# ur-whitelab/nmrgnn

Hardware: AMD Instinct MI355X
Metric: atoms/s (fwd+bwd) on 256-atom/16-neighbor synthetic graphs (higher is better)
Workload: dtype f32 (2xf16-piece MFMA, f32 accumulate)

## Files before the change

include/nmrgnn_hip.h:

```cpp
#ifndef NMRGNN_HIP_H
#define NMRGNN_HIP_H

#include <stdint.h>

#ifdef __cplusplus
extern "C" {
#endif

#define NG_ABI_VERSION 9

enum {
  NG_OK = 0,
  NG_ERR_INVALID = -1,
  NG_ERR_HIP = -2,
  NG_ERR_NOMEM = -3,
  NG_ERR_UNSUPPORTED = -4
};

enum { NG_ACT_NONE = 0, NG_ACT_SOFTPLUS = 1, NG_ACT_RELU = 2, NG_ACT_TANH = 3 };

typedef struct ng_ctx ng_ctx;

int ng_abi_version(void);
int ng_ctx_create(int device, ng_ctx** out);
// ... 78 lines not shown
                const float* dd, float scale, int G, const int32_t* graph_ptr, const float* box, int triclinic, double* strain,
                double* dvec);
int ng_box_grad_csr(ng_ctx*, void* stream, int64_t N, int64_t nnz, const float* pos, const int32_t* row_ptr,
                    const int32_t* col, const float* dd, float scale, int G, const int32_t* graph_ptr, const float* box,
                    int triclinic, double* strain, double* dvec);

int ng_embed_fwd(ng_ctx*, void* stream, int64_t N, int C, int F, const float* atoms,
                 const float* Wemb, float* h0);
int ng_embed_bwd(ng_ctx*, void* stream, int64_t N, int C, int F, const float* atoms,
                 const float* dh0, float* dWemb);

int ng_mp_aggregate(ng_ctx*, void* stream, int64_t N, int K, int F, int E, const float* h,
                    const int32_t* nlist, const float* e, float* A);

int ng_mp_layer_fwd(ng_ctx*, void* stream, int64_t N, int K, int F, int E, int act, int residual,
                    const float* h, const int32_t* nlist, const float* e, const float* inv_degree,
                    const float* w, float* h_out, float* A_save, float* s_save);
int ng_mp_layer_wants_aggregate(int F, int E, int K);

int ng_mp_layer_bwd(ng_ctx*, void* stream, int64_t N, int K, int F, int E, int act,
                    const float* h, const int32_t* nlist, const float* e, const float* inv_degree,
                    const float* w, const float* A_save, const float* s_save,
                    const int32_t* csc_ptr, const int32_t* csc_edge, const float* dh_out,
                    float* dh_in, float* de, int de_accum, float* dw);

int ng_mp_edge_records(ng_ctx*, void* stream, int64_t N, int K, int E, const int32_t* csc_ptr,
                       const int32_t* csc_edge, const float* e, float* rec);
int ng_mp_layer_bwd_rec(ng_ctx*, void* stream, int64_t N, int K, int F, int E, int act,
                    const float* h, const int32_t* nlist, const float* e, const float* inv_degree,
                    const float* w, const float* A_save, const float* s_save,
                    const int32_t* csc_ptr, const int32_t* csc_edge, const float* dh_out,
                    float* dh_in, float* de, int de_accum, float* dw, const float* csc_rec);

int ng_mp_aggregate_csr(ng_ctx*, void* stream, int64_t N, int F, int E, const float* h,
                        const int32_t* row_ptr, const int32_t* col, const float* e, float* A);
int ng_mp_layer_fwd_csr(ng_ctx*, void* stream, int64_t N, int64_t nnz, int F, int E, int act, int residual,
                        const float* h, const int32_t* row_ptr, const int32_t* col, const float* e,
                        const float* inv_degree, const float* w, float* h_out, float* A_save, float* s_save);
int ng_mp_layer_bwd_csr(ng_ctx*, void* stream, int64_t N, int64_t nnz, int F, int E, int act, const float* h,
                        const int32_t* row_ptr, const int32_t* col, const int32_t* row_of, const float* e,
                        const float* inv_degree, const float* w, const float* A_save, const float* s_save,
                        const int32_t* csc_ptr, const int32_t* csc_edge, const float* dh_out, float* dh_in,
                        float* de, int de_accum, float* dw);

int ng_mp_layer_fwd_short(ng_ctx*, void* stream, int64_t N, int K, int F, int E, int act, int residual, const float* h,
                          const int32_t* nlist, const float* e, const float* inv_degree, const float* w, float* h_out);
int ng_mp_layer_fwd_short_csr(ng_ctx*, void* stream, int64_t N, int F, int E, int act, int residual, const float* h,
                              const int32_t* row_ptr, const int32_t* col, const float* e, const float* inv_degree,
                              const float* w, float* h_out);
int ng_mp_layer_short_ok(int64_t N, int K, int F, int E);
int ng_fc_head_ok(int64_t N, int F, int L, int C, int act);
int ng_fc_head_fwd(ng_ctx*, void* stream, int64_t N, int F, int L, int C, int act, const float* x,
                   const float* const* W, const float* const* b, const float* Wout, const float* bout,
                   const float* atoms, const float* pstd, const float* pavg, float* peaks);

int ng_build_incoming_lists(ng_ctx*, void* stream, int64_t N, int K, int64_t n_entries, const int32_t* nlist,
                            const float* edges, int32_t* nlist_c, int32_t* csc_ptr, int32_t* csc_edge);
size_t ng_incoming_lists_scratch_bytes(int64_t N, int64_t n_entries);

int ng_cutoff_count(ng_ctx*, void* stream, int G, int n, float cutoff, const float* pos, int32_t* deg);
int ng_cutoff_fill(ng_ctx*, void* stream, int G, int n, float cutoff, float scale, const float* pos,
                   const int32_t* row_ptr, int32_t* col, float* dist, float* inv_degree);
int ng_cutoff_fill_rows(ng_ctx*, void* stream, int G, int n, float cutoff, float scale, const float* pos,
                        const int32_t* row_ptr, int32_t* col, float* dist, float* inv_degree, int32_t* row_of);
int ng_cutoff_count_pbc(ng_ctx*, void* stream, int G, int n, float cutoff, const float* pos, const float* box, int triclinic,
                        int32_t* deg);
// ... 100 lines not shown
```

nmrgnn_amd/_lib.py:

```python
from __future__ import annotations

import ctypes as C
import os
import threading

_HERE = os.path.dirname(os.path.abspath(__file__))
LIB_PATH = os.environ.get("NMRGNN_HIP_LIB") or os.path.join(_HERE, "csrc", "libnmrgnn_hip.so")

NG_ACT_NONE, NG_ACT_SOFTPLUS, NG_ACT_RELU, NG_ACT_TANH = 0, 1, 2, 3
ACT_CODES = {None: NG_ACT_NONE, "linear": NG_ACT_NONE, "softplus": NG_ACT_SOFTPLUS, "relu": NG_ACT_RELU,
             "tanh": NG_ACT_TANH}

_c_float_p = C.POINTER(C.c_float)
_c_int32_p = C.POINTER(C.c_int32)
_vp = C.c_void_p
_i64 = C.c_int64
_u64 = C.c_uint64
_int = C.c_int
_f = C.c_float

SIGNATURES = {
    "ng_abi_version": (_int, []),
    "ng_ctx_create": (_int, [_int, C.POINTER(_vp)]),
    "ng_ctx_destroy": (None, [_vp]),
# ... 27 lines not shown
    "ng_edge_table_scatter": (_int, [_vp, _vp, _i64, _int, _int, _int, _vp, _vp, _vp, _vp, _vp, _vp]),
    "ng_edge_mlp_bwd": (_int, [_vp, _vp, _i64, _int, _int, _int, _int, _vp, _vp, _vp, _f,
                               C.POINTER(_vp), _vp, _vp, C.POINTER(_vp), C.POINTER(_vp)]),
    "ng_edge_mlp_bwd_tape": (_int, [_vp, _vp, _i64, _int, _int, _int, _int, _vp, _vp, _vp, _f,
                                    C.POINTER(_vp), _vp, _vp, C.POINTER(_vp), C.POINTER(_vp), _int]),
    "ng_build_live_edges": (_int, [_vp, _vp, _i64, _vp, _vp, _vp, _vp, _vp]),
    "ng_build_graph_lists": (_int, [_vp, _vp, _i64, _int, _vp, _vp, _vp, _vp, _vp, _vp, _vp, _vp, _vp]),
    "ng_graph_lists_one_launch": (_int, [_i64, _int]),
    "ng_add_noise_live": (_int, [_vp, _vp, _u64, _u64, _i64, _vp, _vp, _f, _vp, _vp]),
    "ng_edge_live_supported": (_int, [_int, _int, _int, _int]),
    "ng_edge_mlp_fwd_live": (_int, [_vp, _vp, _i64, _int, _int, _int, _int, _vp, _vp, _vp, _vp, _vp, _f,
                                    C.POINTER(_vp), C.POINTER(_vp), _vp, _vp]),
    "ng_edge_mlp_bwd_live": (_int, [_vp, _vp, _i64, _int, _int, _int, _int, _vp, _vp, _vp, _vp, _vp, _f,
                                    C.POINTER(_vp), _vp, _vp, C.POINTER(_vp), C.POINTER(_vp), _int]),
    "ng_edge_mlp_dinput": (_int, [_vp, _vp, _i64, _int, _int, _int, _int, _vp, _vp, _vp, _vp, _vp, _f,
                                  C.POINTER(_vp), C.POINTER(_vp), _vp, _vp, _vp]),
    "ng_positions_grad": (_int, [_vp, _vp, _i64, _int, _vp, _vp, _vp, _vp, _f, _vp, _vp, _vp]),
    "ng_positions_grad_csr": (_int, [_vp, _vp, _i64, _i64, _vp, _vp, _vp, _vp, _vp, _f, _vp, _vp, _vp]),
    "ng_positions_grad_pbc": (_int, [_vp, _vp, _i64, _int, _vp, _vp, _vp, _vp, _f, _vp, _vp, _int, _vp, _int, _vp]),
    "ng_positions_grad_csr_pbc": (_int, [_vp, _vp, _i64, _i64, _vp, _vp, _vp, _vp, _vp, _f, _vp, _vp, _int, _vp, _int, _vp]),
    "ng_box_grad": (_int, [_vp, _vp, _i64, _int, _vp, _vp, _vp, _vp, _f, _int, _vp, _vp, _int, _vp, _vp]),
    "ng_box_grad_csr": (_int, [_vp, _vp, _i64, _i64, _vp, _vp, _vp, _vp, _f, _int, _vp, _vp, _int, _vp, _vp]),
    "ng_restraint_loss": (_int, [_vp, _vp, _int, _i64, _vp, _vp, _vp, _vp, _vp]),
    "ng_restraint_loss_ex": (_int, [_vp, _vp, _int, _i64, _int, _vp, _vp, _vp, _vp, _vp, _f, _vp, _vp, _vp, _vp]),
    "ng_embed_fwd": (_int, [_vp, _vp, _i64, _int, _int, _vp, _vp, _vp]),
    "ng_embed_bwd": (_int, [_vp, _vp, _i64, _int, _int, _vp, _vp, _vp]),
    "ng_mp_aggregate": (_int, [_vp, _vp, _i64, _int, _int, _int, _vp, _vp, _vp, _vp]),
    "ng_mp_layer_fwd": (_int, [_vp, _vp, _i64, _int, _int, _int, _int, _int, _vp, _vp, _vp, _vp, _vp,
                               _vp, _vp, _vp]),
    "ng_mp_layer_bwd": (_int, [_vp, _vp, _i64, _int, _int, _int, _int, _vp, _vp, _vp, _vp, _vp,
                               _vp, _vp, _vp, _vp, _vp, _vp, _vp, _int, _vp]),
    "ng_mp_layer_bwd_rec": (_int, [_vp, _vp, _i64, _int, _int, _int, _int, _vp, _vp, _vp, _vp, _vp,
                               _vp, _vp, _vp, _vp, _vp, _vp, _vp, _int, _vp, _vp]),
    "ng_mp_edge_records": (_int, [_vp, _vp, _i64, _int, _int, _vp, _vp, _vp, _vp]),
    "ng_mp_aggregate_csr": (_int, [_vp, _vp, _i64, _int, _int, _vp, _vp, _vp, _vp, _vp]),
    "ng_mp_layer_fwd_csr": (_int, [_vp, _vp, _i64, _i64, _int, _int, _int, _int, _vp, _vp, _vp, _vp, _vp, _vp,
                                   _vp, _vp, _vp]),
    "ng_mp_layer_bwd_csr": (_int, [_vp, _vp, _i64, _i64, _int, _int, _int, _vp, _vp, _vp, _vp, _vp, _vp, _vp,
                                   _vp, _vp, _vp, _vp, _vp, _vp, _vp, _int, _vp]),
    "ng_build_incoming_lists": (_int, [_vp, _vp, _i64, _int, _i64, _vp, _vp, _vp, _vp, _vp]),
    "ng_incoming_lists_scratch_bytes": (C.c_size_t, [_i64, _i64]),
    "ng_cutoff_count": (_int, [_vp, _vp, _int, _int, _f, _vp, _vp]),
    "ng_cutoff_fill": (_int, [_vp, _vp, _int, _int, _f, _f, _vp, _vp, _vp, _vp, _vp]),
    "ng_cutoff_fill_rows": (_int, [_vp, _vp, _int, _int, _f, _f, _vp, _vp, _vp, _vp, _vp, _vp]),
    "ng_cutoff_count_pbc": (_int, [_vp, _vp, _int, _int, _f, _vp, _vp, _int, _vp]),
    "ng_cutoff_fill_rows_pbc": (_int, [_vp, _vp, _int, _int, _f, _f, _vp, _vp, _int, _vp, _vp, _vp, _vp, _vp]),
    "ng_exclusive_scan_i32": (_int, [_vp, _vp, _i64, _vp, _vp]),
    "ng_dense_fwd": (_int, [_vp, _vp, _i64, _int, _int, _int, _int, _vp, _vp, _vp, _vp, _vp]),
    "ng_dense_bwd": (_int, [_vp, _vp, _i64, _int, _int, _int, _int, _vp, _vp, _vp, _vp, _vp, _vp,
                            _vp]),
    "ng_head_fwd": (_int, [_vp, _vp, _i64, _int, _int, _vp, _vp, _vp, _vp, _vp, _vp, _vp, _vp]),
    "ng_head_fwd_dropout": (_int, [_vp, _vp, _i64, _int, _int, _vp, _u64, _u64, _f, _vp, _vp, _vp, _vp, _vp, _vp, _vp]),
    "ng_head_bwd": (_int, [_vp, _vp, _i64, _int, _int, _vp, _vp, _vp, _vp, _vp, _vp, _vp, _vp, _vp]),
    "ng_head_loss_blocks": (_int, [_vp, _int, _int, _int, _i64]),
    "ng_head_loss_bwd": (_int, [_vp, _vp, _i64, _int, _int, _int, _i64, _vp, _u64, _u64, _f, _vp, _vp, _vp, _vp, _vp, _vp, _vp,
                               _vp, _vp, _f, _vp, _vp, _vp]),
    "ng_head_loss_reduce": (_int, [_vp, _vp, _vp, _int, _int, _int, _vp, _vp, _vp]),
    "ng_mp_layer_wants_aggregate": (_int, [_int, _int, _int]),
    "ng_fc_block_fwd": (_int, [_vp, _vp, _i64, _int, _int, _int, _vp, _vp, _vp, _vp, _vp]),
    "ng_fc_block_scratch_floats": (_i64, [_i64, _int, _int]),
    "ng_fc_block_bwd": (_int, [_vp, _vp, _i64, _int, _int, _int, _vp, _vp, _vp, _vp, _vp, _vp, _vp, _vp]),
    "ng_mp_layer_fwd_short": (_int, [_vp, _vp, _i64, _int, _int, _int, _int, _int, _vp, _vp, _vp, _vp, _vp, _vp]),
    "ng_mp_layer_fwd_short_csr": (_int, [_vp, _vp, _i64, _int, _int, _int, _int, _vp, _vp, _vp, _vp, _vp, _vp, _vp]),
    "ng_mp_layer_short_ok": (_int, [_i64, _int, _int, _int]),
    "ng_fc_head_ok": (_int, [_i64, _int, _int, _int, _int]),
    "ng_fc_head_fwd": (_int, [_vp, _vp, _i64, _int, _int, _int, _int, _vp, C.POINTER(_vp), C.POINTER(_vp), _vp, _vp, _vp,
# ... 119 lines not shown
```

nmrgnn_amd/engine.py:

```python
from __future__ import annotations

import ctypes as C
import os

import numpy as np
import torch

from . import _lib
from ._lib import ptr, ptr_array
from .graph import GraphBatch
from .params import ParamStore

ACT = {None: 0, "linear": 0, "softplus": 1, "relu": 2, "tanh": 3}
DROPOUT_RATE = 0.2
FUSED_TAIL_MAX_ATOMS = 16384


def rbf_grid(low, high, count):
    lo, hi = np.float32(low), np.float32(high)
    delta = (hi - lo) / np.float32(count - 1)
    c = (lo + delta * np.arange(count, dtype=np.float32)).astype(np.float32)
    c[-1] = hi
    return c, float(np.float32(c[1] - c[0]))


def edge_path(edge_table, use_live_edges, live_kernels, E, n_edges, min_edges, is_csr, capturing):
    fits = n_edges * E * 4 < (1 << 31)
    sized = edge_table and E <= 8 and n_edges >= min_edges and fits
    if live_kernels and fits:
        return "table" if sized else ("live" if use_live_edges else "slots")
    if sized and not is_csr and not capturing:
        return "table_host"
    return "slots"


class Tape:
    __slots__ = ("batch", "d_eff", "z_save", "z_layout", "e", "h", "A", "S", "fx", "g", "drop_mask",
                 "peaks", "edge_path", "live", "table", "loss", "dpeaks", "dg", "head_partial")


class Engine:
    _ids = 0

    def __init__(self, hp, num_elem, peak_std=None, peak_avg=None, device=None, seed=1234):
        if not torch.cuda.is_available():
            raise _lib.NGError("nmrgnn_amd needs an AMD GPU (torch.cuda.is_available() is False); "
                               "there is no CPU fallback")
        if device is None:
            device = torch.device("cuda", torch.cuda.current_device())
        self.device = torch.device(device)
        if self.device.index is None:
            self.device = torch.device("cuda", torch.cuda.current_device())
        self.ctx = _lib.get_context(self.device.index)
        self.lib = self.ctx.lib
        self.hp = hp
        self.C = int(num_elem)
        self.F = hp.get('atom_feature_size')
        self.E = hp.get('edge_feature_size')
        self.H = hp.get('edge_hidden_size')
        self.L = hp.get('mp_layers')
        self.Le = hp.get('edge_fc_layers')
        self.Lf = hp.get('fc_layers')
        self.sigma = float(hp.get('noise'))
        self.use_dropout = bool(hp.get('dropout'))
        if hp.get('fc_activation') not in ACT or hp.get('mp_activation') not in ACT:
            raise ValueError(f"unsupported activation {hp.get('fc_activation')!r} / {hp.get('mp_activation')!r}")
        self.fc_act = ACT[hp.get('fc_activation')]
        self.mp_act = ACT[hp.get('mp_activation')]
        self.params = ParamStore(hp, self.C, self.device, seed=seed)
        self.params.on_change = self._on_params_changed
        c, gap = rbf_grid(hp.get('rbf_low'), hp.get('rbf_high'), self.H)
        self.centers = torch.from_numpy(c).to(self.device)
        self.gap = gap
        std = np.ones(self.C, np.float32) if peak_std is None else np.asarray(peak_std, np.float32)[:self.C]
        avg = np.zeros(self.C, np.float32) if peak_avg is None else np.asarray(peak_avg, np.float32)[:self.C]
        self.peak_std = torch.from_numpy(np.ascontiguousarray(std)).to(self.device)
        self.peak_avg = torch.from_numpy(np.ascontiguousarray(avg)).to(self.device)
        self.adam_m = torch.zeros_like(self.params.flat)
        self.adam_v = torch.zeros_like(self.params.flat)
        self.adam_t = 0
        self.tape = None
        self._rng_calls = 0
        self._frozen = False
        self.cache_images = False
        self.defer_reductions = True
        self.fuse_head_loss = os.environ.get("NG_HEAD_LOSS", "1") != "0"
        self.use_live_edges = os.environ.get("NG_EDGE_LIVE", "1") != "0"
        self.edge_table = os.environ.get("NG_EDGE_TABLE", "1") != "0"
        self.edge_table_tol = 3.0e-6
        self.edge_table_min_edges = 262144
        self.edge_table_force_fallback = False
        self._wgen = 0
        self._table_cache = None
        self._rows_2t = torch.full((1,), 2 * self._table_points(), dtype=torch.int32, device=self.device)
        Engine._ids += 1
        self._id = Engine._ids

    def freeze_weights(self, on=True):
        self._frozen = bool(on)
        if not on:
            self._ck(self.lib.ng_weights_frozen(self.ctx.handle, 0), "ng_weights_frozen")

    def weights_changed(self):
        self._wgen += 1
        self._ck(self.lib.ng_weights_changed(self.ctx.handle), "ng_weights_changed")

    def _on_params_changed(self):
        self._wgen += 1
        self.lib.ng_weights_changed(self.ctx.handle)

    def _st(self):
        return C.c_void_p(torch.cuda.current_stream(self.device).cuda_stream)

    def _new(self, *shape):
        return torch.empty(*shape, dtype=torch.float32, device=self.device)

    def _ck(self, rc, what):
        self.ctx.check(rc, what)

    def randn(self, n, seed, offset=0):
        out = self._new(n)
        self._ck(self.lib.ng_randn(self.ctx.handle, self._st(), seed, offset, ptr(out), n), "ng_randn")
        return out

    def dropout_mask(self, n, seed, offset=0, keep=1.0 - DROPOUT_RATE):
        out = self._new(n)
        self._ck(self.lib.ng_dropout_mask(self.ctx.handle, self._st(), seed, offset, keep, ptr(out), n),
                 "ng_dropout_mask")
        return out

    def forward(self, batch: GraphBatch, training=False, noise=None, dropout_mask=None, seed=0, keep_tape=None, loss=None):
        if loss is not None and not (training if keep_tape is None else keep_tape):
            raise ValueError("forward(loss=...) needs a tape (training=True)")
        if not (self._frozen or self.cache_images):
            return self._forward(batch, training, noise, dropout_mask, seed, keep_tape, loss)
        self._ck(self.lib.ng_weights_frozen(self.ctx.handle, self._id), "ng_weights_frozen")
        try:
            return self._forward(batch, training, noise, dropout_mask, seed, keep_tape, loss)
        finally:
            self.lib.ng_weights_frozen(self.ctx.handle, 0)

    def _forward(self, batch, training, noise, dropout_mask, seed, keep_tape=None, loss=None):
        tape = bool(training) if keep_tape is None else bool(keep_tape)
        lib, h, st = self.lib, self.ctx.handle, self._st()
        P = self.params
        N, K, F, E, H = batch.N, batch.K, self.F, self.E, self.H
        if batch.C != self.C:
            raise ValueError(f"atoms has {batch.C} element columns, model was built for {self.C}")
        ne = batch.n_edges
        self._ck(lib.ng_ctx_set_graph_span(h, batch.max_graph_atoms), "ng_ctx_set_graph_span")
        d_src = batch.edges.reshape(-1)
        d_eff = d_src
        live_kernels = bool(lib.ng_edge_live_supported(H, E, self.Le, self.fc_act))
        path = edge_path(self.edge_table, self.use_live_edges, live_kernels, E, ne, self.edge_table_min_edges, batch.is_csr,
                         torch.cuda.is_current_stream_capturing())
        live = batch.live_edges(force=path == "table") if path in ("table", "live") else None
        if live is None and path in ("table", "live"):
            path = "slots"
        perm = pos = rows = None
        if live is not None:
            perm, pos, d_c, rows = live
            d_src = d_eff = d_c
            if training and self.sigma > 0:
                d_eff = self._new(ne)
                self._ck(lib.ng_add_noise_live(h, st, seed, 0, ne, ptr(batch.edges), ptr(None if noise is None else noise.reshape(-1)),
                                               self.sigma, ptr(pos), ptr(d_eff)), "ng_add_noise_live")
        elif training and self.sigma > 0:
            d_eff = self._new(ne)
            if noise is None:
                self._ck(lib.ng_add_noise(h, st, seed, 0, ne, ptr(d_src), self.sigma, ptr(d_eff)), "ng_add_noise")
            else:
                noise = noise.reshape(-1)
                self._ck(lib.ng_add_scaled(h, st, ne, ptr(d_src), ptr(noise), self.sigma, ptr(d_eff)),
                         "ng_add_scaled")
        table = self._edge_table_build(batch, live, d_eff, tape, training) if path in ("table", "table_host") else None
        if path == "table_host" and table is None:
            path = "slots"
        if path == "table":
            rows = table["gate"][1:]
        e = self._new(ne, E)
        z_save, z_layout = None, 0
        if path != "table_host":
            z_save, z_layout = self._edge_mlp_fwd(ne, d_src, d_eff, e, tape, perm, rows)
        if table is not None:
            self._ck(lib.ng_edge_table_interp(h, st, ne, E, table["T"], ptr(batch.edges), ptr(d_eff), ptr(pos),
                                              ptr(table["rng"]), ptr(table["e_all"]), ptr(table["gate"]), ptr(e)),
                     "ng_edge_table_interp")
        h0 = self._new(N, F)
        self._ck(lib.ng_embed_fwd(h, st, N, self.C, F, ptr(batch.atoms), ptr(P["embed/kernel"]),
                                  ptr(h0)), "ng_embed_fwd")
        hs, As, Ss = [h0], [], []
        for l in range(self.L):
            hn = self._new(N, F)
            S = self._new(N, F) if (tape and self.mp_act != 0) else None
            if batch.is_csr and not tape and N <= FUSED_TAIL_MAX_ATOMS and lib.ng_mp_layer_short_ok(N, 1, F, E):
                A = None
                self._ck(lib.ng_mp_layer_fwd_short_csr(h, st, N, F, E, self.mp_act, 1, ptr(hs[-1]), ptr(batch.row_ptr),
                                                       ptr(batch.nlist), ptr(e), ptr(batch.inv_degree), ptr(P[f"mp/{l}/w"]),
                                                       ptr(hn)), "ng_mp_layer_fwd_short_csr")
            elif batch.is_csr:
                A = self._new(N, E, F) if tape else None
                self._ck(lib.ng_mp_layer_fwd_csr(h, st, N, ne, F, E, self.mp_act, 1, ptr(hs[-1]),
                                                 ptr(batch.row_ptr), ptr(batch.nlist), ptr(e),
                                                 ptr(batch.inv_degree), ptr(P[f"mp/{l}/w"]), ptr(hn), ptr(A),
                                                 ptr(S)), "ng_mp_layer_fwd_csr")
            elif not tape and N <= FUSED_TAIL_MAX_ATOMS and lib.ng_mp_layer_short_ok(N, K, F, E):
                A = None
                self._ck(lib.ng_mp_layer_fwd_short(h, st, N, K, F, E, self.mp_act, 1, ptr(hs[-1]), ptr(batch.nlist_c), ptr(e),
                                                   ptr(batch.inv_degree), ptr(P[f"mp/{l}/w"]), ptr(hn)), "ng_mp_layer_fwd_short")
            else:
                A = self._new(N, E, F) if (tape and lib.ng_mp_layer_wants_aggregate(F, E, K)) else None
                self._ck(lib.ng_mp_layer_fwd(h, st, N, K, F, E, self.mp_act, 1, ptr(hs[-1]),
                                             ptr(batch.nlist_c), ptr(e), ptr(batch.inv_degree),
                                             ptr(P[f"mp/{l}/w"]), ptr(hn), ptr(A), ptr(S)),
                         "ng_mp_layer_fwd")
            hs.append(hn)
            As.append(A)
            Ss.append(S)
        Wfc = [P[f"fc/{t}/kernel"] for t in range(self.Lf)]
        Bfc = [P[f"fc/{t}/bias"] for t in range(self.Lf)]
        if not tape and not (training and self.use_dropout) and N <= FUSED_TAIL_MAX_ATOMS \
                and lib.ng_fc_head_ok(N, F, self.Lf, self.C, self.fc_act):
            peaks = self._new(N)
            self._ck(lib.ng_fc_head_fwd(h, st, N, F, self.Lf, self.C, self.fc_act, ptr(hs[-1]), ptr_array(Wfc), ptr_array(Bfc),
                                        ptr(P["out/kernel"]), ptr(P["out/bias"]), ptr(batch.atoms), ptr(self.peak_std),
                                        ptr(self.peak_avg), ptr(peaks)), "ng_fc_head_fwd")
            return peaks
        fx = [hs[-1]]
# ... 11 lines not shown
            nb = int(lib.ng_head_loss_blocks(h, batch.G, Fh, self.C, batch.max_graph_atoms))
        if nb > 0:
            y, w, gw = loss
            keep = (1.0 - DROPOUT_RATE) if (training and self.use_dropout) else 1.0
            loss_t, dg = self._new(1), self._new(N, Fh)
            head_partial = self._new(nb, Fh * self.C + self.C + 1)
            self._ck(lib.ng_head_loss_bwd(h, st, N, batch.G, Fh, self.C, batch.max_graph_atoms, ptr(g), seed, 1 << 40, keep,
                                          None, ptr(P["out/kernel"]), ptr(P["out/bias"]), ptr(batch.atoms),
                                          ptr(self.peak_std), ptr(self.peak_avg), ptr(batch.graph_ptr), ptr(y), ptr(w),
                                          float(gw), ptr(peaks), ptr(dg), ptr(head_partial)),
                     "ng_head_loss_bwd")
        elif training and self.use_dropout and dropout_mask is None:
            mask = self._new(N, Fh)
            self._ck(lib.ng_head_fwd_dropout(h, st, N, Fh, self.C, ptr(g), seed, 1 << 40, 1.0 - DROPOUT_RATE, ptr(mask),
                                             ptr(P["out/kernel"]), ptr(P["out/bias"]), ptr(batch.atoms),
                                             ptr(self.peak_std), ptr(self.peak_avg), ptr(peaks)), "ng_head_fwd_dropout")
        else:
            if training and self.use_dropout:
                mask = dropout_mask.reshape(N, Fh).contiguous()
            self._ck(lib.ng_head_fwd(h, st, N, Fh, self.C, ptr(g), ptr(mask), ptr(P["out/kernel"]),
                                     ptr(P["out/bias"]), ptr(batch.atoms), ptr(self.peak_std),
                                     ptr(self.peak_avg), ptr(peaks)), "ng_head_fwd")
        if loss is not None and nb == 0:
            y, w, gw = loss
            loss_t, dpeaks = self.loss_l2(batch, y, w, peaks)
            if gw != 1.0:
                dpeaks.mul_(gw)
        if tape:
            tp = Tape()
            tp.loss, tp.dpeaks, tp.dg, tp.head_partial = loss_t, dpeaks, dg, head_partial
            tp.batch, tp.d_eff, tp.z_save, tp.e = batch, d_eff, z_save, e
            tp.z_layout = z_layout
            tp.edge_path, tp.live, tp.table = path, live, table
            tp.h, tp.A, tp.S, tp.fx, tp.g, tp.drop_mask, tp.peaks = hs, As, Ss, fx, g, mask, peaks
            self.tape = tp
        return peaks

    EDGE_TABLE_POINTS = 4096

    def _table_points(self):
        return self.EDGE_TABLE_POINTS if self.E <= 4 else self.EDGE_TABLE_POINTS // 2

    def _edge_weights(self):
        P = self.params
        return [P[f"edge_fc/{t}/kernel"] for t in range(self.Le)], [P[f"edge_fc/{t}/bias"] for t in range(self.Le)]

    def _edge_grads(self, view=None):
        view = view or self.params.g
        return [view(f"edge_fc/{t}/kernel") for t in range(self.Le)], [view(f"edge_fc/{t}/bias") for t in range(self.Le)]

    def _edge_mlp_fwd(self, n, d_src, d_eff, e, tape, perm=None, rows=None):
        lib, h, st = self.lib, self.ctx.handle, self._st()
        z, z_layout = None, 0
        if tape:
            z = self._new(self.Le - 1, n, self.H)
            z_layout = int(lib.ng_edge_tape_layout(self.H, self.E, self.Le, self.fc_act, n))
        W, B = self._edge_weights()
        if perm is None:
            self._ck(lib.ng_edge_mlp_fwd(h, st, n, self.H, self.E, self.Le, self.fc_act, ptr(d_src), ptr(d_eff), ptr(self.centers),
                                         self.gap, ptr_array(W), ptr_array(B), ptr(e), ptr(z)), "ng_edge_mlp_fwd")
        else:
            self._ck(lib.ng_edge_mlp_fwd_live(h, st, n, self.H, self.E, self.Le, self.fc_act, ptr(d_src), ptr(d_eff), ptr(perm),
                                              ptr(rows), ptr(self.centers), self.gap, ptr_array(W), ptr_array(B), ptr(e), ptr(z)),
                     "ng_edge_mlp_fwd_live")
        return z, z_layout

# ... 102 lines not shown
                     "ng_head_loss_reduce")
        else:
            if tp.dg is not None:
                raise RuntimeError("backward(dpeaks) after forward(loss=...): the head's backward already ran with the "
                                   "loss gradient; call backward(None)")
            if dpeaks is None:
                dpeaks = tp.dpeaks
            if dpeaks is None:
                raise RuntimeError("backward(None) without forward(loss=...)")
            dpeaks = dpeaks.contiguous()
            dg = self._new(N, Fh)
            self._ck(lib.ng_head_bwd(h, st, N, Fh, self.C, ptr(tp.g), ptr(tp.drop_mask),
                                     ptr(P["out/kernel"]), ptr(b.atoms), ptr(self.peak_std),
                                     ptr(dpeaks), ptr(dg), ptr(wg("out/kernel")), ptr(wg("out/bias"))),
                     "ng_head_bwd")
        dx = self._new(N, F)
        Wfc = [P[f"fc/{t}/kernel"] for t in range(self.Lf)]
        ns = int(lib.ng_fc_block_scratch_floats(N, F, self.Lf))
        scratch = self._new(ns) if ns else None
        self._ck(lib.ng_fc_block_bwd(h, st, N, F, self.Lf, self.fc_act, ptr_array(tp.fx), ptr(tp.g),
                                     ptr_array(Wfc), ptr(dg), ptr(dx),
                                     warr([wg(f"fc/{t}/kernel") for t in range(self.Lf)]),
                                     warr([wg(f"fc/{t}/bias") for t in range(self.Lf)]),
                                     ptr(scratch)), "ng_fc_block_bwd")
        csc_ptr, csc_edge = b.csc()
        de = self._new(ne, E)
        rec = None
        if E <= 3 and not b.is_csr:
            rec = self._new(ne, 4)
            self._ck(lib.ng_mp_edge_records(h, st, N, K, E, ptr(csc_ptr), ptr(csc_edge), ptr(tp.e), ptr(rec)),
                     "ng_mp_edge_records")
        dh = dx
        for l in reversed(range(self.L)):
            dhn = self._new(N, F)
            if b.is_csr:
                self._ck(lib.ng_mp_layer_bwd_csr(h, st, N, ne, F, E, self.mp_act, ptr(tp.h[l]), ptr(b.row_ptr),
                                                 ptr(b.nlist), ptr(b.row_of), ptr(tp.e), ptr(b.inv_degree),
                                                 ptr(P[f"mp/{l}/w"]), ptr(tp.A[l]), ptr(tp.S[l]), ptr(csc_ptr),
                                                 ptr(csc_edge), ptr(dh), ptr(dhn), ptr(de),
                                                 0 if l == self.L - 1 else 1, ptr(wg(f"mp/{l}/w"))),
                         "ng_mp_layer_bwd_csr")
                dh = dhn
                continue
            self._ck(lib.ng_mp_layer_bwd_rec(h, st, N, K, F, E, self.mp_act, ptr(tp.h[l]), ptr(b.nlist_c),
                                         ptr(tp.e), ptr(b.inv_degree), ptr(P[f"mp/{l}/w"]),
                                         ptr(tp.A[l]), ptr(tp.S[l]), ptr(csc_ptr), ptr(csc_edge),
                                         ptr(dh), ptr(dhn), ptr(de), 0 if l == self.L - 1 else 1,
                                         ptr(wg(f"mp/{l}/w")), ptr(rec)), "ng_mp_layer_bwd")
            dh = dhn
        if not param_grad:
            self._edge_dinput(tp, de, edge_grad)
            self.tape = None
            return
        self._ck(lib.ng_embed_bwd(h, st, N, self.C, F, ptr(b.atoms), ptr(dh),
                                  ptr(P.g("embed/kernel"))), "ng_embed_bwd")
        self._ck(lib.ng_flush_reductions(h, st), "ng_flush_reductions")
        if on_node_grads is not None:
            on_node_grads()
        if tp.edge_path == "slots":
            self._edge_mlp_bwd(ne, b.edges, tp.d_eff, tp.z_save, tp.z_layout, de, self._edge_grads())
        elif tp.edge_path == "live":
            perm, _, d_c, n_live = tp.live
            self._edge_mlp_bwd(ne, d_c, tp.d_eff, tp.z_save, tp.z_layout, de, self._edge_grads(), perm, n_live)
        elif tp.edge_path == "table_host":
            self._edge_table_backward(tp, de, self._edge_grads())
        else:
            names = [f"edge_fc/{t}/{k}" for t in range(self.Le) for k in ("kernel", "bias")]
            o0 = min(P.offsets[n] for n in names)
            o1 = max(P.offsets[n] + int(np.prod(P.shapes[n])) for n in names)
            tmp = self._new(o1 - o0)
            tv = lambda n: tmp[P.offsets[n] - o0:P.offsets[n] - o0 + int(np.prod(P.shapes[n]))]
            perm, _, d_c, _ = tp.live
            self._edge_mlp_bwd(ne, d_c, tp.d_eff, tp.z_save, tp.z_layout, de, self._edge_grads(tv), perm, tp.table["gate"][1:])
            self._edge_table_backward(tp, de, self._edge_grads())
            blk = P.grad[o0:o1]
            self._ck(lib.ng_add_scaled(h, st, o1 - o0, ptr(blk), ptr(tmp), 1.0, ptr(blk)), "ng_add_scaled")
        if edge_grad is not None:
            self._edge_dinput(tp, de, edge_grad)
        self.tape = None

    def _edge_dinput(self, tp, de, out):
        b = tp.batch
        W, B = self._edge_weights()
        if tp.live is not None:
            perm, _, d_src, n_live = tp.live
        else:
            perm = n_live = None
            d_src = b.edges.reshape(-1)
# ... 38 lines not shown
```

Before: 43.67 million.

## Fuse embedding into first message-passing layer via low-rank atom-feature aggregation

Adds a fused embed+layer-0 path for fwd and bwd. It aggregates raw one-hot atom features (C<=16) times edge features into a small E*C tensor per atom instead of gathering 64-wide embeddings. The combined weight Wemb·w is precomputed in LDS. This avoids materialising h0, the separate embed kernels, and wide neighbor gathers in layer 0. The cost is extra weight-building work per block, a partial-sum reduction kernel for dw/dWemb, and shape limits (F=64, E<=3, K<=16, C<=16).

```diff
diff --git a/include/nmrgnn_hip.h b/include/nmrgnn_hip.h
--- a/include/nmrgnn_hip.h
+++ b/include/nmrgnn_hip.h
@@ -134,6 +134,15 @@
                     const int32_t* csc_ptr, const int32_t* csc_edge, const float* dh_out,
                     float* dh_in, float* de, int de_accum, float* dw, const float* csc_rec);
 
+int ng_mp_embed_layer_ok(int F, int E, int K, int C);
+int ng_mp_embed_layer_fwd(ng_ctx*, void* stream, int64_t N, int K, int F, int E, int C, int act, int residual,
+                          const float* atoms, const float* Wemb, const int32_t* nlist, const float* e,
+                          const float* inv_degree, const float* w, float* h_out, float* s_save, float* T_save);
+int ng_mp_embed_layer_bwd(ng_ctx*, void* stream, int64_t N, int K, int F, int E, int C, int act, int residual,
+                          const float* atoms, const float* Wemb, const int32_t* nlist, const float* e,
+                          const float* inv_degree, const float* w, const float* s_save, const float* T_save,
+                          const float* dh_out, float* de, int de_accum, float* dw, float* dWemb);
+
 int ng_mp_aggregate_csr(ng_ctx*, void* stream, int64_t N, int F, int E, const float* h,
                         const int32_t* row_ptr, const int32_t* col, const float* e, float* A);
 int ng_mp_layer_fwd_csr(ng_ctx*, void* stream, int64_t N, int64_t nnz, int F, int E, int act, int residual,
diff --git a/nmrgnn_amd/_lib.py b/nmrgnn_amd/_lib.py
--- a/nmrgnn_amd/_lib.py
+++ b/nmrgnn_amd/_lib.py
@@ -83,6 +83,11 @@
                                _vp, _vp, _vp, _vp, _vp, _vp, _vp, _int, _vp]),
     "ng_mp_layer_bwd_rec": (_int, [_vp, _vp, _i64, _int, _int, _int, _int, _vp, _vp, _vp, _vp, _vp,
                                _vp, _vp, _vp, _vp, _vp, _vp, _vp, _int, _vp, _vp]),
+    "ng_mp_embed_layer_ok": (_int, [_int, _int, _int, _int]),
+    "ng_mp_embed_layer_fwd": (_int, [_vp, _vp, _i64, _int, _int, _int, _int, _int, _int, _vp, _vp, _vp, _vp, _vp, _vp,
+                                     _vp, _vp, _vp]),
+    "ng_mp_embed_layer_bwd": (_int, [_vp, _vp, _i64, _int, _int, _int, _int, _int, _int, _vp, _vp, _vp, _vp, _vp, _vp,
+                                     _vp, _vp, _vp, _vp, _int, _vp, _vp]),
     "ng_mp_edge_records": (_int, [_vp, _vp, _i64, _int, _int, _vp, _vp, _vp, _vp]),
     "ng_mp_aggregate_csr": (_int, [_vp, _vp, _i64, _int, _int, _vp, _vp, _vp, _vp, _vp]),
     "ng_mp_layer_fwd_csr": (_int, [_vp, _vp, _i64, _i64, _int, _int, _int, _int, _vp, _vp, _vp, _vp, _vp, _vp,
diff --git a/nmrgnn_amd/csrc/mp_embed0.hip b/nmrgnn_amd/csrc/mp_embed0.hip
--- /dev/null
+++ b/nmrgnn_amd/csrc/mp_embed0.hip
@@ -0,0 +1,461 @@
+#include "ng_common.h"
+#include "ng_internal.h"
+#include "mfma_gemm.cuh"
+
+namespace ng {
+namespace {
+
+constexpr int EF = 64;
+constexpr int ETILE = 64;
+constexpr int ENT = 256;
+constexpr int EMAX_E = 3, EMAX_C = 16, EMAX_K = 16;
+constexpr int ROW = EF + 4;
+constexpr int FWD_WGS_PER_CU = 3, BWD_WGS_PER_CU = 2;
+
+struct Shape {
+  int E, C, K;
+  int EC;
+  int ECp;
+  int XS;
+  int GS;
+};
+
+__host__ __device__ inline Shape make_shape(int E, int C, int K) {
+  Shape s;
+  s.E = E; s.C = C; s.K = K;
+  s.EC = E * C;
+  s.ECp = (s.EC + 3) & ~3;
+  s.XS = s.ECp + ((C + 3) & ~3);
+  s.GS = s.EC | 1;
+  return s;
+}
+
+__device__ __forceinline__ void fma4(float4& acc, float x, const float4& m) {
+  acc.x = fmaf(x, m.x, acc.x); acc.y = fmaf(x, m.y, acc.y); acc.z = fmaf(x, m.z, acc.z); acc.w = fmaf(x, m.w, acc.w);
+}
+__device__ __forceinline__ float dot4(const float4& a, const float4& b, float acc) {
+  return fmaf(a.w, b.w, fmaf(a.z, b.z, fmaf(a.y, b.y, fmaf(a.x, b.x, acc))));
+}
+
+__device__ void build_weights(const Shape& s, const float* __restrict__ Wemb, const float* __restrict__ w, float* Ws) {
+  const int tid = threadIdx.x;
+  for (int t = tid; t < s.XS * ROW; t += ENT) Ws[t] = 0.f;
+  __syncthreads();
+  for (int t = tid; t < s.C * EF; t += ENT) Ws[(s.ECp + t / EF) * ROW + (t % EF)] = Wemb[t];
+  const int EFn = s.E * EF;
+  if (tid < EFn) {
+    const int m = tid / s.E, n = tid % s.E;
+    float wv[EF];
+#pragma unroll
+    for (int l = 0; l < EF; ++l) wv[l] = w[(int64_t)l * EFn + tid];
+    for (int c = 0; c < s.C; ++c) {
+      const float* we = Wemb + c * EF;
+      float a0 = 0.f, a1 = 0.f, a2 = 0.f, a3 = 0.f;
+#pragma unroll
+      for (int l = 0; l < EF; l += 4) {
+        a0 = fmaf(we[l], wv[l], a0); a1 = fmaf(we[l + 1], wv[l + 1], a1);
+        a2 = fmaf(we[l + 2], wv[l + 2], a2); a3 = fmaf(we[l + 3], wv[l + 3], a3);
+      }
+      Ws[(n * s.C + c) * ROW + m] = (a0 + a1) + (a2 + a3);
+    }
+  }
+  __syncthreads();
+}
+
+__device__ __forceinline__ void gather_rows(const Shape& s, int64_t N, int64_t tile0, const float* __restrict__ atoms,
+                                            const int32_t* __restrict__ nlist, const float* __restrict__ e,
+                                            const float* __restrict__ T_in, float* Xs) {
+  const int tid = threadIdx.x, al = tid >> 2, q = tid & 3;
+  const int64_t i = tile0 + al;
+  float acc[EMAX_E][4], av[4];
+#pragma unroll
+  for (int n = 0; n < EMAX_E; ++n)
+#pragma unroll
+    for (int u = 0; u < 4; ++u) acc[n][u] = 0.f;
+#pragma unroll
+  for (int u = 0; u < 4; ++u) av[u] = 0.f;
+  if (i < N) {
+#pragma unroll
+    for (int u = 0; u < 4; ++u)
+      if (q + 4 * u < s.C) av[u] = atoms[i * s.C + q + 4 * u];
+    if (T_in) {
+#pragma unroll
+      for (int n = 0; n < EMAX_E; ++n)
+#pragma unroll
+        for (int u = 0; u < 4; ++u)
+          if (n < s.E && q + 4 * u < s.C) acc[n][u] = T_in[i * s.EC + n * s.C + q + 4 * u];
+    } else {
+      const int lim = (int)N - 1;
+      for (int jb = 0; jb < s.K; jb += 8) {
+        int32_t src[8];
+        float ev[8][EMAX_E], sv[8][4];
+        const int32_t* nl = nlist + i * s.K + jb;
+        const float* ep = e + (i * s.K + jb) * s.E;
+#pragma unroll
+        for (int j = 0; j < 8; ++j) src[j] = jb + j < s.K ? nl[j] : 0;
+#pragma unroll
+        for (int j = 0; j < 8; ++j)
+#pragma unroll
+          for (int n = 0; n < EMAX_E; ++n) ev[j][n] = (jb + j < s.K && n < s.E) ? ep[j * s.E + n] : 0.f;
+#pragma unroll
+        for (int j = 0; j < 8; ++j) {
+          const float* row = atoms + (__mul24(min(max(src[j], 0), lim), s.C) + q);
+#pragma unroll
+          for (int u = 0; u < 4; ++u) sv[j][u] = q + 4 * u < s.C ? row[4 * u] : 0.f;
+        }
+#pragma unroll
+        for (int j = 0; j < 8; ++j)
+#pragma unroll
+          for (int n = 0; n < EMAX_E; ++n)
+#pragma unroll
+            for (int u = 0; u < 4; ++u) acc[n][u] = fmaf(ev[j][n], sv[j][u], acc[n][u]);
+      }
+    }
+  }
+  float* x = Xs + al * s.XS;
+#pragma unroll
+  for (int u = 0; u < 4; ++u)
+    if (q + 4 * u < s.C) {
+      x[s.ECp + q + 4 * u] = av[u];
+#pragma unroll
+      for (int n = 0; n < EMAX_E; ++n)
+        if (n < s.E) x[n * s.C + q + 4 * u] = acc[n][u];
+    }
+}
+
+template <int NU>
+__device__ __forceinline__ void g_rows(const Shape& s, const float* d, const float* Ws, float* g_out, int q) {
+  float g[NU];
+  int wr[NU];
+#pragma unroll
+  for (int u = 0; u < NU; ++u) { g[u] = 0.f; wr[u] = min(q + 4 * u, s.ECp - 1) * ROW; }
+#pragma unroll 2
+  for (int m4 = 0; m4 < EF / 4; ++m4) {
+    const float4 dv = *reinterpret_cast<const float4*>(d + 4 * m4);
+#pragma unroll
+    for (int u = 0; u < NU; ++u) g[u] = dot4(dv, *reinterpret_cast<const float4*>(Ws + wr[u] + 4 * m4), g[u]);
+  }
+#pragma unroll
+  for (int u = 0; u < NU; ++u)
+    if (q + 4 * u < s.EC) g_out[q + 4 * u] = g[u];
+}
+
+__device__ __forceinline__ void tile_range(int64_t ntiles, int64_t& t0, int64_t& t1) {
+  t0 = (int64_t)blockIdx.x * ntiles / gridDim.x;
+  t1 = ((int64_t)blockIdx.x + 1) * ntiles / gridDim.x;
+}
+
+__global__ __launch_bounds__(ENT, 3) void mp_embed0_fwd_kernel(Shape s, int64_t N, int act, int residual,
+                                                            const float* __restrict__ atoms, const float* __restrict__ Wemb,
+                                                            const int32_t* __restrict__ nlist, const float* __restrict__ e,
+                                                            const float* __restrict__ inv_degree, const float* __restrict__ w,
+                                                            float* __restrict__ h_out, float* __restrict__ s_save,
+                                                            float* __restrict__ T_save) {
+  extern __shared__ __attribute__((aligned(16))) float lds[];
+  float* Ws = lds;
+  float* Xs = lds + s.XS * ROW;
+  const int tid = threadIdx.x;
+  build_weights(s, Wemb, w, Ws);
+  for (int t = tid; t < ETILE * s.XS; t += ENT) Xs[t] = 0.f;
+  const int ta = tid >> 4, tm = tid & 15;
+  int64_t t0, t1;
+  tile_range((N + ETILE - 1) / ETILE, t0, t1);
+  for (int64_t tile = t0; tile < t1; ++tile) {
+    const int64_t a0 = tile * ETILE;
+    __syncthreads();
+    gather_rows(s, N, a0, atoms, nlist, e, nullptr, Xs);
+    __syncthreads();
+    if (T_save) {
+      const int64_t lim = (N - a0 < ETILE ? N - a0 : ETILE) * s.EC;
+      for (int t = tid; t < lim; t += ENT) T_save[a0 * s.EC + t] = Xs[(t / s.EC) * s.XS + (t % s.EC)];
+    }
+    float4 accP[4], accR[4];
+#pragma unroll
+    for (int a = 0; a < 4; ++a) { accP[a] = f4zero(); accR[a] = f4zero(); }
+    for (int k = 0; k < s.XS; k += 4) {
+      float4 x[4], m[4];
+#pragma unroll
+      for (int a = 0; a < 4; ++a) x[a] = *reinterpret_cast<const float4*>(Xs + (4 * ta + a) * s.XS + k);
+#pragma unroll
+      for (int r = 0; r < 4; ++r) m[r] = *reinterpret_cast<const float4*>(Ws + (k + r) * ROW + 4 * tm);
+      if (k < s.ECp) {
+#pragma unroll
+        for (int a = 0; a < 4; ++a) { fma4(accP[a], x[a].x, m[0]); fma4(accP[a], x[a].y, m[1]); fma4(accP[a], x[a].z, m[2]); fma4(accP[a], x[a].w, m[3]); }
+      } else if (residual) {
+#pragma unroll
+        for (int a = 0; a < 4; ++a) { fma4(accR[a], x[a].x, m[0]); fma4(accR[a], x[a].y, m[1]); fma4(accR[a], x[a].z, m[2]); fma4(accR[a], x[a].w, m[3]); }
+      }
+    }
+#pragma unroll
+    for (int a = 0; a < 4; ++a) {
+      const int64_t i = a0 + 4 * ta + a;
+      if (i < N) {
+        const float inv = inv_degree[i];
+        float4 sv;
+        sv.x = act_apply(act, inv * accP[a].x); sv.y = act_apply(act, inv * accP[a].y);
+        sv.z = act_apply(act, inv * accP[a].z); sv.w = act_apply(act, inv * accP[a].w);
+        if (s_save) *reinterpret_cast<float4*>(s_save + i * EF + 4 * tm) = sv;
+        *reinterpret_cast<float4*>(h_out + i * EF + 4 * tm) =
+            make_float4(sv.x + accR[a].x, sv.y + accR[a].y, sv.z + accR[a].z, sv.w + accR[a].w);
+      }
+    }
+  }
+}
+
+__global__ __launch_bounds__(ENT, 2) void mp_embed0_bwd_kernel(Shape s, int64_t N, int act, int residual,
+                                                            const float* __restrict__ atoms, const float* __restrict__ Wemb,
+                                                            const int32_t* __restrict__ nlist, const float* __restrict__ e,
+                                                            const float* __restrict__ inv_degree, const float* __restrict__ w,
+                                                            const float* __restrict__ s_save, const float* __restrict__ T_in,
+                                                            const float* __restrict__ dh_out, float* __restrict__ de,
+                                                            int de_accum, float* __restrict__ partial) {
+  extern __shared__ __attribute__((aligned(16))) float lds[];
+  float* Ws = lds;
+  float* Xs = Ws + s.XS * ROW;
+  float* dPs = Xs + ETILE * s.XS;
+  float* dHs = dPs + ETILE * ROW;
+  float* Gs = dHs + ETILE * ROW;
+  const int tid = threadIdx.x;
+  build_weights(s, Wemb, w, Ws);
+  for (int t = tid; t < ETILE * s.XS; t += ENT) Xs[t] = 0.f;
+  const int tr = tid >> 4, tm = tid & 15;
+  const int al = tid >> 2, q = tid & 3;
+  const bool want_w = partial != nullptr;
+  const bool q_rows = 4 * tr < s.ECp, r_rows = 4 * tr >= s.ECp && 4 * tr < s.XS && residual;
+  const float* Ys = q_rows ? dPs : dHs;
+  float4 acc[4];
+#pragma unroll
+  for (int r = 0; r < 4; ++r) acc[r] = f4zero();
+  const int nu = s.ECp >> 2;
+  int64_t t0, t1;
+  tile_range((N + ETILE - 1) / ETILE, t0, t1);
+  for (int64_t tile = t0; tile < t1; ++tile) {
+    const int64_t a0 = tile * ETILE;
+    __syncthreads();
+    for (int t = tid; t < ETILE * (EF / 4); t += ENT) {
+      const int a = t >> 4, c4 = t & 15;
+      const int64_t i = a0 + a;
+      float4 dh = f4zero(), dp = f4zero();
+      if (i < N) {
+        dh = *reinterpret_cast<const float4*>(dh_out + i * EF + 4 * c4);
+        const float inv = inv_degree[i];
+        float4 g = make_float4(1.f, 1.f, 1.f, 1.f);
+        if (act != 0) {
+          const float4 sv = *reinterpret_cast<const float4*>(s_save + i * EF + 4 * c4);
+          g = make_float4(act_grad_from_out(act, sv.x), act_grad_from_out(act, sv.y), act_grad_from_out(act, sv.z),
+                          act_grad_from_out(act, sv.w));
+        }
+        dp = make_float4(dh.x * g.x * inv, dh.y * g.y * inv, dh.z * g.z * inv, dh.w * g.w * inv);
+      }
+      *reinterpret_cast<float4*>(dPs + a * ROW + 4 * c4) = dp;
+      *reinterpret_cast<float4*>(dHs + a * ROW + 4 * c4) = dh;
+    }
+    if (want_w) gather_rows(s, N, a0, atoms, nlist, e, T_in, Xs);
+    __syncthreads();
+    if (nu <= 4) g_rows<4>(s, dPs + al * ROW, Ws, Gs + al * s.GS, q);
+    else if (nu <= 8) g_rows<8>(s, dPs + al * ROW, Ws, Gs + al * s.GS, q);
+    else g_rows<12>(s, dPs + al * ROW, Ws, Gs + al * s.GS, q);
+    __syncthreads();
+    {
+      const int64_t i = a0 + al;
+      if (i < N) {
+        const float* gi = Gs + al * s.GS;
+        int32_t src[EMAX_K / 4];
+        float row[EMAX_K / 4][EMAX_C], sum[EMAX_K / 4][EMAX_E];
+#pragma unroll
+        for (int u = 0; u < EMAX_K / 4; ++u) src[u] = q + 4 * u < s.K ? nlist[i * s.K + q + 4 * u] : 0;
+#pragma unroll
+        for (int u = 0; u < EMAX_K / 4; ++u)
+#pragma unroll
+          for (int n = 0; n < EMAX_E; ++n)
+            sum[u][n] = (de_accum && q + 4 * u < s.K && n < s.E) ? de[(i * s.K + q + 4 * u) * s.E + n] : 0.f;
+#pragma unroll
+        for (int u = 0; u < EMAX_K / 4; ++u) {
+          const float* rp = atoms + __mul24(min(max(src[u], 0), (int)N - 1), s.C);
+#pragma unroll
+          for (int c = 0; c < EMAX_C; ++c) row[u][c] = c < s.C ? rp[c] : 0.f;
+        }
+        for (int n = 0; n < s.E; ++n) {
+          float part[EMAX_K / 4];
+#pragma unroll
+          for (int u = 0; u < EMAX_K / 4; ++u) part[u] = 0.f;
+#pragma unroll
+          for (int c = 0; c < EMAX_C; ++c) {
+            const float gv = gi[min(n * s.C + c, s.EC - 1)];
+#pragma unroll
+            for (int u = 0; u < EMAX_K / 4; ++u) part[u] = fmaf(gv, row[u][c], part[u]);
+          }
+#pragma unroll
+          for (int u = 0; u < EMAX_K / 4; ++u) {
+            const float prior = n == 0 ? sum[u][0] : (n == 1 ? sum[u][1] : sum[u][2]);
+            if (q + 4 * u < s.K) de[(i * s.K + q + 4 * u) * s.E + n] = prior + part[u];
+          }
+        }
+      }
+    }
+    if (want_w && (q_rows || r_rows)) {
+      for (int a = 0; a < ETILE; ++a) {
+        const float4 x = *reinterpret_cast<const float4*>(Xs + a * s.XS + 4 * tr);
+        const float4 y = *reinterpret_cast<const float4*>(Ys + a * ROW + 4 * tm);
+        fma4(acc[0], x.x, y); fma4(acc[1], x.y, y); fma4(acc[2], x.z, y); fma4(acc[3], x.w, y);
+      }
+    }
+  }
+  if (want_w) {
+    float* out = partial + (int64_t)blockIdx.x * (s.EC + s.C) * EF;
+#pragma unroll
+    for (int r = 0; r < 4; ++r) {
+      const int row = 4 * tr + r;
+      int orow = -1;
+      if (row < s.EC) orow = row;
+      else if (row >= s.ECp && row < s.ECp + s.C) orow = s.EC + row - s.ECp;
+      if (orow >= 0) *reinterpret_cast<float4*>(out + orow * EF + 4 * tm) = acc[r];
+    }
+  }
+}
+
+constexpr int FNT = 1024;
+
+template <int SLOTS, class Off>
+__device__ __forceinline__ void sum_partials(const float* __restrict__ partial, int nz, int64_t zstride, int nslots, Off off,
+                                             float4* red, float4* S) {
+  constexpr int ZL = FNT / SLOTS;
+  const int tid = threadIdx.x, slot = tid % SLOTS, zl = tid / SLOTS;
+  float4 acc = f4zero();
+  if (slot < nslots) {
+    const float* p = partial + off(slot);
+    int z = zl;
+    for (; z + 15 * ZL < nz; z += 16 * ZL) {
+      float4 v[16];
+#pragma unroll
+      for (int u = 0; u < 16; ++u) v[u] = *reinterpret_cast<const float4*>(p + (int64_t)(z + u * ZL) * zstride);
+#pragma unroll
+      for (int u = 0; u < 16; ++u) { acc.x += v[u].x; acc.y += v[u].y; acc.z += v[u].z; acc.w += v[u].w; }
+    }
+    for (; z < nz; z += ZL) {
+      const float4 v = *reinterpret_cast<const float4*>(p + (int64_t)z * zstride);
+      acc.x += v.x; acc.y += v.y; acc.z += v.z; acc.w += v.w;
+    }
+  }
+  red[tid] = acc;
+  __syncthreads();
+  if (tid < SLOTS) {
+    float4 t = red[tid];
+    for (int k = 1; k < ZL; ++k) { const float4 v = red[k * SLOTS + tid]; t.x += v.x; t.y += v.y; t.z += v.z; t.w += v.w; }
+    S[tid] = t;
+  }
+  __syncthreads();
+}
+
+__global__ __launch_bounds__(FNT) void mp_embed0_finish_kernel(Shape s, int nz, int residual, const float* __restrict__ partial,
+                                                               const float* __restrict__ Wemb, const float* __restrict__ w,
+                                                               float* __restrict__ dw, float* __restrict__ dWemb) {
+  __shared__ float4 red[FNT];
+  __shared__ float4 S4[64];
+  const float* S = reinterpret_cast<const float*>(S4);
+  const int tid = threadIdx.x, b = blockIdx.x;
+  const int64_t zstride = (int64_t)(s.EC + s.C) * EF;
+  if (b < 8 * s.E) {
+    const int n = b >> 3, m0 = 8 * (b & 7);
+    sum_partials<32>(partial, nz, zstride, 2 * s.C, [&](int slot) { return (n * s.C + (slot >> 1)) * EF + m0 + 4 * (slot & 1); },
+                     red, S4);
+    if (tid < EF * 8) {
+      const int l = tid >> 3, mm = tid & 7;
+      float sum = 0.f;
+      for (int c = 0; c < s.C; ++c) sum = fmaf(Wemb[c * EF + l], S[c * 8 + mm], sum);
+      dw[((int64_t)l * EF + m0 + mm) * s.E + n] = sum;
+    }
+  } else {
+    const int c = b - 8 * s.E;
+    sum_partials<64>(partial, nz, zstride, 16 * (s.E + 1),
+                     [&](int slot) { const int r = slot >> 4; return (r < s.E ? r * s.C + c : s.EC + c) * EF + 4 * (slot & 15); },
+                     red, S4);
+    const int l = tid >> 4, part = tid & 15;
+    const int per = 4 * s.E;
+    float sum = 0.f;
+    for (int t = part * per; t < (part + 1) * per; ++t) {
+      const int m = t / s.E, n = t % s.E;
+      sum = fmaf(S[n * EF + m], w[(int64_t)l * EF * s.E + t], sum);
+    }
+    float* redf = reinterpret_cast<float*>(red);
+    redf[tid] = sum;
+    __syncthreads();
+    if (part == 0) {
+      float t = residual ? S[s.E * EF + l] : 0.f;
+      for (int k = 0; k < 16; ++k) t += redf[tid + k];
+      dWemb[c * EF + l] = t;
+    }
+  }
+}
+
+inline size_t fwd_lds(const Shape& s) { return (size_t)(s.XS * ROW + ETILE * s.XS) * 4; }
+inline size_t bwd_lds(const Shape& s) { return (size_t)(s.XS * ROW + ETILE * s.XS + 2 * ETILE * ROW + ETILE * s.GS) * 4; }
+inline int grid_for(const ng_ctx* ctx, int64_t N, int wgs_per_cu) {
+  return (int)std::max<int64_t>(1, std::min<int64_t>(cdiv(N, ETILE), (int64_t)ctx->num_cu * wgs_per_cu));
+}
+
+}
+}
+
+using namespace ng;
+
+extern "C" int ng_mp_embed_layer_ok(int F, int E, int K, int C) {
+  return F == EF && E >= 1 && E <= EMAX_E && K >= 1 && K <= 16 && C >= 1 && C <= EMAX_C;
+}
+
+extern "C" int ng_mp_embed_layer_fwd(ng_ctx* ctx, void* stream, int64_t N, int K, int F, int E, int C, int act, int residual,
+                                     const float* atoms, const float* Wemb, const int32_t* nlist, const float* e,
+                                     const float* inv_degree, const float* w, float* h_out, float* s_save, float* T_save) {
+  if (!ctx) return NG_ERR_INVALID;
+  if (!ng_mp_embed_layer_ok(F, E, K, C)) { ctx->err = "mp_embed_layer: F == 64, E <= 3, K <= 16, C <= 16"; return NG_ERR_UNSUPPORTED; }
+  NG_REQUIRE(ctx, N >= 0 && N < (1 << 24), "mp_embed_layer_fwd: at most 2^24 - 1 atoms per call (24-bit row arithmetic in the gather)");
+  NG_REQUIRE(ctx, act >= 0 && act <= 3, "mp_embed_layer_fwd: activation code");
+  if (N == 0) return NG_OK;
+  NG_REQUIRE(ctx, atoms && Wemb && nlist && e && inv_degree && w && h_out, "mp_embed_layer_fwd: arguments");
+  const Shape s = make_shape(E, C, K);
+  ProfScope ps(ctx, (hipStream_t)stream, "mp_win_fwd");
+  hipLaunchKernelGGL(mp_embed0_fwd_kernel, dim3(grid_for(ctx, N, FWD_WGS_PER_CU)), dim3(ENT), fwd_lds(s), (hipStream_t)stream, s, N, act,
+                     residual, atoms, Wemb, nlist, e, inv_degree, w, h_out, s_save, T_save);
+  NG_HIP(ctx, hipGetLastError());
+  return NG_OK;
+}
+
+extern "C" int ng_mp_embed_layer_bwd(ng_ctx* ctx, void* stream, int64_t N, int K, int F, int E, int C, int act, int residual,
+                                     const float* atoms, const float* Wemb, const int32_t* nlist, const float* e,
+                                     const float* inv_degree, const float* w, const float* s_save, const float* T_save,
+                                     const float* dh_out, float* de, int de_accum, float* dw, float* dWemb) {
+  if (!ctx) return NG_ERR_INVALID;
+  hipStream_t st = (hipStream_t)stream;
+  if (!ng_mp_embed_layer_ok(F, E, K, C)) { ctx->err = "mp_embed_layer: F == 64, E <= 3, K <= 16, C <= 16"; return NG_ERR_UNSUPPORTED; }
+  NG_REQUIRE(ctx, N >= 0 && N < (1 << 24), "mp_embed_layer_bwd: at most 2^24 - 1 atoms per call (24-bit row arithmetic in the gather)");
+  NG_REQUIRE(ctx, act >= 0 && act <= 3, "mp_embed_layer_bwd: activation code");
+  NG_REQUIRE(ctx, (dw == nullptr) == (dWemb == nullptr), "mp_embed_layer_bwd: dw and dWemb are both given or both NULL");
+  NG_REQUIRE(ctx, act == NG_ACT_NONE || s_save, "mp_embed_layer_bwd: s_save required for an activation");
+  if (N == 0) {
+    if (dw) {
+      NG_HIP(ctx, hipMemsetAsync(dw, 0, (size_t)F * F * E * 4, st));
+      NG_HIP(ctx, hipMemsetAsync(dWemb, 0, (size_t)C * F * 4, st));
+    }
+    return NG_OK;
+  }
+  NG_REQUIRE(ctx, atoms && Wemb && nlist && e && inv_degree && w && dh_out && de, "mp_embed_layer_bwd: arguments");
+  const Shape s = make_shape(E, C, K);
+  const int grid = grid_for(ctx, N, BWD_WGS_PER_CU);
+  float* partial = nullptr;
+  if (dw) {
+    partial = (float*)workspace(ctx, (size_t)grid * (s.EC + s.C) * EF * 4);
+    if (!partial) return NG_ERR_NOMEM;
+  }
+  {
+    ProfScope ps(ctx, st, "mp_win_bwd_edge");
+    hipLaunchKernelGGL(mp_embed0_bwd_kernel, dim3(grid), dim3(ENT), bwd_lds(s), st, s, N, act, residual, atoms, Wemb, nlist, e,
+                       inv_degree, w, s_save, T_save, dh_out, de, de_accum, partial);
+    NG_HIP(ctx, hipGetLastError());
+  }
+  if (dw) {
+    ProfScope ps(ctx, st, "mp_embed0_finish");
+    hipLaunchKernelGGL(mp_embed0_finish_kernel, dim3(8 * E + C), dim3(FNT), 0, st, s, grid, residual, partial, Wemb, w, dw, dWemb);
+    NG_HIP(ctx, hipGetLastError());
+  }
+  return NG_OK;
+}
diff --git a/nmrgnn_amd/engine.py b/nmrgnn_amd/engine.py
--- a/nmrgnn_amd/engine.py
+++ b/nmrgnn_amd/engine.py
@@ -36,7 +36,7 @@
 
 class Tape:
     __slots__ = ("batch", "d_eff", "z_save", "z_layout", "e", "h", "A", "S", "fx", "g", "drop_mask",
-                 "peaks", "edge_path", "live", "table", "loss", "dpeaks", "dg", "head_partial")
+                 "peaks", "edge_path", "live", "table", "loss", "dpeaks", "dg", "head_partial", "embed0")
 
 
 class Engine:
@@ -86,6 +86,7 @@
         self.defer_reductions = True
         self.fuse_head_loss = os.environ.get("NG_HEAD_LOSS", "1") != "0"
         self.use_live_edges = os.environ.get("NG_EDGE_LIVE", "1") != "0"
+        self.embed0 = os.environ.get("NG_MP_EMBED0", "1") != "0"
         self.edge_table = os.environ.get("NG_EDGE_TABLE", "1") != "0"
         self.edge_table_tol = 3.0e-6
         self.edge_table_min_edges = 262144
@@ -128,6 +129,12 @@
         self._ck(self.lib.ng_dropout_mask(self.ctx.handle, self._st(), seed, offset, keep, ptr(out), n),
                  "ng_dropout_mask")
         return out
+
+    def _embed0_path(self, batch):
+        lib, K = self.lib, batch.K
+        return bool(self.embed0 and self.L >= 1 and not batch.is_csr
+                    and lib.ng_mp_embed_layer_ok(self.F, self.E, K, self.C)
+                    and not lib.ng_mp_layer_wants_aggregate(self.F, self.E, K))
 
     def forward(self, batch: GraphBatch, training=False, noise=None, dropout_mask=None, seed=0, keep_tape=None, loss=None):
         if loss is not None and not (training if keep_tape is None else keep_tape):
@@ -186,14 +193,22 @@
             self._ck(lib.ng_edge_table_interp(h, st, ne, E, table["T"], ptr(batch.edges), ptr(d_eff), ptr(pos),
                                               ptr(table["rng"]), ptr(table["e_all"]), ptr(table["gate"]), ptr(e)),
                      "ng_edge_table_interp")
-        h0 = self._new(N, F)
-        self._ck(lib.ng_embed_fwd(h, st, N, self.C, F, ptr(batch.atoms), ptr(P["embed/kernel"]),
-                                  ptr(h0)), "ng_embed_fwd")
+        embed0 = self._embed0_path(batch)
+        h0 = None
+        if not embed0:
+            h0 = self._new(N, F)
+            self._ck(lib.ng_embed_fwd(h, st, N, self.C, F, ptr(batch.atoms), ptr(P["embed/kernel"]),
+                                      ptr(h0)), "ng_embed_fwd")
         hs, As, Ss = [h0], [], []
         for l in range(self.L):
             hn = self._new(N, F)
             S = self._new(N, F) if (tape and self.mp_act != 0) else None
-            if batch.is_csr and not tape and N <= FUSED_TAIL_MAX_ATOMS and lib.ng_mp_layer_short_ok(N, 1, F, E):
+            if l == 0 and embed0:
+                A = torch.empty(N, E, self.C, dtype=torch.float32, device=self.device) if tape else None
+                self._ck(lib.ng_mp_embed_layer_fwd(h, st, N, K, F, E, self.C, self.mp_act, 1, ptr(batch.atoms),
+                                                   ptr(P["embed/kernel"]), ptr(batch.nlist_c), ptr(e), ptr(batch.inv_degree),
+                                                   ptr(P["mp/0/w"]), ptr(hn), ptr(S), ptr(A)), "ng_mp_embed_layer_fwd")
+            elif batch.is_csr and not tape and N <= FUSED_TAIL_MAX_ATOMS and lib.ng_mp_layer_short_ok(N, 1, F, E):
                 A = None
                 self._ck(lib.ng_mp_layer_fwd_short_csr(h, st, N, F, E, self.mp_act, 1, ptr(hs[-1]), ptr(batch.row_ptr),
                                                        ptr(batch.nlist), ptr(e), ptr(batch.inv_degree), ptr(P[f"mp/{l}/w"]),
@@ -271,6 +286,7 @@
             tp.batch, tp.d_eff, tp.z_save, tp.e = batch, d_eff, z_save, e
             tp.z_layout = z_layout
             tp.edge_path, tp.live, tp.table = path, live, table
+            tp.embed0 = embed0
             tp.h, tp.A, tp.S, tp.fx, tp.g, tp.drop_mask, tp.peaks = hs, As, Ss, fx, g, mask, peaks
             self.tape = tp
         return peaks
@@ -439,6 +455,13 @@
                      "ng_mp_edge_records")
         dh = dx
         for l in reversed(range(self.L)):
+            if l == 0 and tp.embed0:
+                self._ck(lib.ng_mp_embed_layer_bwd(h, st, N, K, F, E, self.C, self.mp_act, 1, ptr(b.atoms),
+                                                   ptr(P["embed/kernel"]), ptr(b.nlist_c), ptr(tp.e), ptr(b.inv_degree),
+                                                   ptr(P["mp/0/w"]), ptr(tp.S[0]), ptr(tp.A[0]), ptr(dh), ptr(de),
+                                                   0 if self.L == 1 else 1, ptr(wg("mp/0/w")), ptr(wg("embed/kernel"))),
+                         "ng_mp_embed_layer_bwd")
+                break
             dhn = self._new(N, F)
             if b.is_csr:
                 self._ck(lib.ng_mp_layer_bwd_csr(h, st, N, ne, F, E, self.mp_act, ptr(tp.h[l]), ptr(b.row_ptr),
@@ -459,8 +482,9 @@
             self._edge_dinput(tp, de, edge_grad)
             self.tape = None
             return
-        self._ck(lib.ng_embed_bwd(h, st, N, self.C, F, ptr(b.atoms), ptr(dh),
-                                  ptr(P.g("embed/kernel"))), "ng_embed_bwd")
+        if not tp.embed0:
+            self._ck(lib.ng_embed_bwd(h, st, N, self.C, F, ptr(b.atoms), ptr(dh),
+                                      ptr(P.g("embed/kernel"))), "ng_embed_bwd")
         self._ck(lib.ng_flush_reductions(h, st), "ng_flush_reductions")
         if on_node_grads is not None:
             on_node_grads()
```

Result: no change. 43.69 million, median of 6 (+0.0%).
